# tooHotSpot/FGN

Hardware: AMD Instinct MI355X
Metric: query-imgs/sec (3-way 3-shot, 800x1333 FGN simple_test) (higher is better)
Workload: dtype f32; 1 GPU; cfg3: COCO2VOC 3-way 3-shot, query 3x800x1333, supports 9x3x256^2, ResNet-50-C4, R<=300 proposals, D<=100 detections, 1 episode(s) per GPU per step; h2d_in_step=True, gt_mask_rle_in_step=True, world_size_seen=1, phase_lock=rpn, caller_streams=2, support_cache=False, hip_graph=True, winograd_3x3=F(4x4,3x3)

## Files before the change

### fgn_amd/csrc/conv_igemm.hip

```cpp
#include "common.h"
#include <cstdlib>

struct ConvParams {
    const float* x = nullptr;
    const float* w = nullptr;
    float* y = nullptr;
    const float* scale = nullptr;
    const float* shift = nullptr;
    const float* residual = nullptr;
    const float* in_scale = nullptr;
    const int32_t* n_img_dev = nullptr;
    int n_img = 0, H = 1, W = 1, Cin = 0, Ho = 1, Wo = 1, Cout = 0, KH = 1, KW = 1, stride = 1, pad = 0;
    int a_img_div = 1;
    int relu = 0;
    int K = 0;
    int n_tiles_n = 0;
    int band_nt = 0, band_mt = 0;
    float* ws = nullptr;
    int splits = 1, kt_per_split = 0;
#ifdef FGN_EXPERIMENTS
    int32_t* tickets = nullptr;
    int32_t* sched = nullptr;
    int sk_U = 0, sk_dp = 0;
#endif
// ... 1152 lines not shown
    int tiles[2];
    const float* xs[2] = {x0, x1};
    float* ys[2] = {y0, y1};
    const int ns[2] = {n_img0, n_img1}, Hs[2] = {H0, H1}, Ws[2] = {W0, W1};
    for (int i = 0; i < 2; ++i) {
        const ConvPlan g = conv_geometry(ns[i], Hs[i], Ws[i], Cin, Cout, cout_pad, KH, KW, stride, pad, 1);
        if (g.rc != FGN_OK || g.x_bytes == 0) return FGN_ERR_SHAPE;
        ConvParams& p = ps[i];
        p.x = xs[i]; p.w = w_packed; p.y = ys[i]; p.scale = scale; p.shift = shift;
        p.n_img = ns[i]; p.H = Hs[i]; p.W = Ws[i]; p.Cin = Cin; p.Cout = Cout; p.KH = KH; p.KW = KW;
        p.stride = stride; p.pad = pad; p.relu = relu;
        p.Ho = g.Ho; p.Wo = g.Wo; p.K = g.K; p.x_bytes = g.x_bytes; p.w_bytes = g.w_bytes;
        p.kt_per_split = p.K / BK;
        p.n_tiles_n = cdiv(Cout, 64);
        const int m_tiles = cdiv((int)g.M, 64);
        set_band(p, 64, m_tiles, 64ll * p.K * 4);
        tiles[i] = (m_tiles * p.n_tiles_n + 7) / 8 * 8;
    }
    constexpr int NST = CONV_DMA_STAGES;
    const size_t dlds = std::max((size_t)NST * (64 + 64) * BK, (size_t)64 * (64 + 4)) * sizeof(float);
    const dim3 grid(tiles[0] + tiles[1]), wg(256);
    return Cin != 4 ? launch_kernel<conv_igemm_dma_pair_kernel<64, 64, 32, 32, NST, 4, 0>>(grid, wg, dlds, stream, ps[0], ps[1], tiles[0])
                    : launch_kernel<conv_igemm_dma_pair_kernel<64, 64, 32, 32, NST, 4, 2>>(grid, wg, dlds, stream, ps[0], ps[1], tiles[0]);
}

static int x3_pick_bm(long long M, int Cout, int K, int grp_rows, int grp_valid, int bm) {
    if (bm == 64 || bm == 128) return (grp_rows && grp_rows % bm) ? 0 : bm;
    if (grp_rows && grp_rows % 64) return 0;
    const int nt = cdiv(Cout, X3_BN);
    if (Cout * 10 < nt * X3_BN * 7) return 0;
    if (((M + 63) / 64) * nt < 192) return 0;
    const long long groups = grp_rows ? M / grp_rows : 1;
    const long long valid = grp_rows ? std::min<long long>(grp_valid > 0 ? grp_valid : grp_rows, grp_rows) : M;
    const long long rows64 = (valid + 63) / 64 * 64, rows128 = (valid + 127) / 128 * 128;
    if (K >= 256 && (!grp_rows || grp_rows % 128 == 0) && rows128 * 100 <= rows64 * 108 && groups * (rows128 / 128) * nt >= 400)
        return 128;
    return 64;
}

template <int WMW, int RB, int NT, int NST, bool SH16>
static int launch_x3_cfg(ConvParams& p, int M_max, hipStream_t stream) {
    constexpr int BM = 32 * RB * WMW;
    const int m_tiles = cdiv(M_max, BM);
    set_band(p, BM, m_tiles, (long long)X3_BN * p.K * 6);
    const int tiles = m_tiles * p.n_tiles_n;
    static unsigned long long ok = 0ull;
    hipError_t attr = fgn_allow_full_lds(reinterpret_cast<const void*>(conv_pw_x3_kernel<WMW, RB, NT, NST, SH16>), &ok);
    if (attr != hipSuccess) return (int)attr;
    const size_t lds = (size_t)NST * (BM * 128 + X3_B_STAGE);
    const int per_cu = (int)(160 * 1024 / lds);
    const int grid = std::min(256 * per_cu, (tiles + 7) / 8 * 8);
    p.stamp = fgn_next_stamp_record();
    FGN_LAUNCH_TIMED((conv_pw_x3_kernel<WMW, RB, NT, NST, SH16>), dim3(grid), dim3(128 * WMW), lds, stream, p, tiles);
    FGN_LAUNCH_CHECK();
    return FGN_OK;
}

static int launch_x3(const ConvParams& p0, int M_max, int bm, int nterms, hipStream_t stream) {
    ConvParams p = p0;
    if (!p.w3 || p.npad3 % X3_BN || p.npad3 < p.Cout || (p.Cout & 3) || p.K % BK || p.K < 2 * BK || p.splits != 1) return FGN_ERR_SHAPE;
    p.n_tiles_n = cdiv(p.Cout, X3_BN);
#ifdef FGN_EXPERIMENTS
    if (bm >= 2000) {
        const int b = bm - 2000;
        if (x3_pick_bm(M_max, p.Cout, p.K, p.grp_rows, p.grp_valid, b == 129 ? 128 : b) == 0) return FGN_ERR_SHAPE;
        if (b == 129) return nterms == 9 ? launch_x3_cfg<4, 1, 9, 3, false>(p, M_max, stream) : launch_x3_cfg<4, 1, 6, 3, false>(p, M_max, stream);
        if (b == 128) return launch_x3_cfg<2, 2, 6, 2, false>(p, M_max, stream);
        if (b == 64) return nterms == 9 ? launch_x3_cfg<2, 1, 9, 2, false>(p, M_max, stream) : launch_x3_cfg<2, 1, 6, 2, false>(p, M_max, stream);
        return FGN_ERR_SHAPE;
    }
#endif
    if (bm != 0 && bm != 64 && bm != 128) return FGN_ERR_SHAPE;
    const int BM = x3_pick_bm(M_max, p.Cout, p.K, p.grp_rows, p.grp_valid, bm);
    if (BM == 0) return FGN_ERR_SHAPE;
    if (nterms == 9) return BM == 64 ? launch_x3_cfg<2, 1, 9, 2, true>(p, M_max, stream) : FGN_ERR_SHAPE;
    return BM == 128 ? launch_x3_cfg<2, 2, 6, 2, true>(p, M_max, stream) : launch_x3_cfg<2, 1, 6, 2, true>(p, M_max, stream);
}

extern "C" size_t fgn_x3_image_bytes(int K, int npad, int n_groups) { return (size_t)n_groups * K * npad * 6; }
extern "C" int fgn_x3_row_tile(long long M, int Cout, int K, int grp_rows, int grp_valid) {
    return x3_pick_bm(M, Cout, K, grp_rows, grp_valid, 0);
}

#ifdef X3_PHASES
static unsigned long long* g_x3_ph = nullptr;
extern "C" int fgn_x3_phases(unsigned long long* host16) {
    if (!g_x3_ph) return FGN_ERR_ARG;
    if (hipDeviceSynchronize() != hipSuccess) return FGN_ERR_ARG;
    if (hipMemcpy(host16, g_x3_ph, 128, hipMemcpyDeviceToHost) != hipSuccess) return FGN_ERR_ARG;
    return hipMemset(g_x3_ph, 0, 128) == hipSuccess ? FGN_OK : FGN_ERR_ARG;
}
#endif

static int h2_pick(long long M, int Cout, int K, int grp_rows, int grp_valid, int bm) {
    if (bm == 264) return (grp_rows && grp_rows % 128) ? 0 : 264;
    if (bm != 0) return x3_pick_bm(M, Cout, K, grp_rows, grp_valid, bm);
    if (Cout <= 64) {
        if (grp_rows && grp_rows % 128) return 0;
        if (Cout < 48 || (M + 127) / 128 < 256) return 0;
        return 264;
    }
    const int bm_x3 = x3_pick_bm(M, Cout, K, grp_rows, grp_valid, 0);
    return (bm_x3 == 128 && !grp_rows) ? 64 : bm_x3;
}

template <int WMW, int WNW, int RB, int NST, bool IM2COL, int KG = 1>
static int launch_h2_cfg(ConvParams& p, const H2Im2col& q2, int M_max, hipStream_t stream) {
    constexpr int BM = 32 * RB * WMW, BN = 64 * WNW;
    const int m_tiles = cdiv(M_max, BM);
    p.n_tiles_n = cdiv(p.Cout, BN);
    set_band(p, BM, m_tiles, (long long)BN * p.K * 4);
    const int tiles = m_tiles * p.n_tiles_n;
    static unsigned long long ok = 0ull;
    hipError_t attr = fgn_allow_full_lds(reinterpret_cast<const void*>(conv_pw_h2_kernel<WMW, WNW, RB, NST, IM2COL, KG>), &ok);
    if (attr != hipSuccess) return (int)attr;
    const size_t lds = (size_t)KG * NST * (BM * 128 + 2 * BN * 64);
    const int per_cu = std::min(3, (int)(160 * 1024 / lds));
    const int grid = std::min(256 * per_cu, (tiles + 7) / 8 * 8);
    p.stamp = fgn_next_stamp_record();
    FGN_LAUNCH_TIMED((conv_pw_h2_kernel<WMW, WNW, RB, NST, IM2COL, KG>), dim3(grid), dim3(64 * WMW * WNW * KG), lds, stream, p, q2, tiles);
    FGN_LAUNCH_CHECK();
    return FGN_OK;
}

extern "C" size_t fgn_h2_image_bytes(int K, int npad, int n_groups) { return (size_t)n_groups * npad * ((size_t)K * 4 + 4); }
extern "C" int fgn_h2_row_tile(long long M, int Cout, int K, int grp_rows, int grp_valid) {
    return h2_pick(M, Cout, K, grp_rows, grp_valid, 0);
}

constexpr int H2_KG_MIN_KTILES = 8;
constexpr int H2_BM_KG2 = 1064;
extern "C" int fgn_h2_k_groups(long long M, int Cout, int K, int grp_rows, int grp_valid) {
    if (h2_pick(M, Cout, K, grp_rows, grp_valid, 0) != 64 || grp_rows != 0 || K % BK) return 1;
    const int kt = K / BK;
    if ((kt & 1) || kt < H2_KG_MIN_KTILES) return 1;
    return cdiv(M, 64) * (long long)cdiv(Cout, H2_BN) <= 256 ? 2 : 1;
}

static int launch_h2(const ConvParams& p0, int M_max, int n_groups, int bm, hipStream_t stream, const H2Im2col* im = nullptr) {
    ConvParams p = p0;
    if (!p.w3 || p.npad3 % H2_BN || p.npad3 < p.Cout || (p.Cout & 3) || p.K % BK || p.K < 2 * BK || p.splits != 1) return FGN_ERR_SHAPE;
    const size_t img = (size_t)n_groups * p.K * p.npad3 * 4;
    p.w3_bytes = (unsigned)img;
    p.w_inv = reinterpret_cast<const float*>(static_cast<const char*>(p.w3) + img);
    H2Im2col none;
    none.y1 = nullptr; none.x_off0 = none.x_off1 = 0u; none.M0 = none.M1 = 0; none.H1 = none.W1 = none.Ho1 = none.Wo1 = 1; none.cin_shift = 0;
    if (bm != 0 && bm != 64 && bm != 128 && bm != 264 && bm != H2_BM_KG2) return FGN_ERR_SHAPE;
    if (bm == H2_BM_KG2 && ((p.K / BK) % 2 || p.K / BK < 4)) return FGN_ERR_SHAPE;
    const int cfg = h2_pick(M_max, p.Cout, p.K, p.grp_rows, p.grp_valid, bm == H2_BM_KG2 ? 64 : bm);
    if (cfg == 0) return FGN_ERR_SHAPE;
    const int kgroups = bm == H2_BM_KG2 ? 2 : (bm == 0 ? fgn_h2_k_groups(M_max, p.Cout, p.K, p.grp_rows, p.grp_valid) : 1);
    if (kgroups == 2)
        return im ? launch_h2_cfg<2, 2, 1, 2, true, 2>(p, *im, M_max, stream) : launch_h2_cfg<2, 2, 1, 2, false, 2>(p, none, M_max, stream);
    if (im) {
        if (cfg == 264) return launch_h2_cfg<4, 1, 1, 2, true>(p, *im, M_max, stream);
        return cfg == 128 ? launch_h2_cfg<2, 2, 2, 2, true>(p, *im, M_max, stream) : launch_h2_cfg<2, 2, 1, 2, true>(p, *im, M_max, stream);
    }
    if (cfg == 264) return launch_h2_cfg<4, 1, 1, 2, false>(p, none, M_max, stream);
    return cfg == 128 ? launch_h2_cfg<2, 2, 2, 2, false>(p, none, M_max, stream) : launch_h2_cfg<2, 2, 1, 2, false>(p, none, M_max, stream);
}

extern "C" int fgn_conv2d_pair_h2_bm_nhwc_f32(const float* x0, int n_img0, int H0, int W0, const float* x1, int n_img1, int H1,
                                              int W1, const void* w_h2, float* y0, float* y1, const float* scale,
                                              const float* shift, int Cin, int Cout, int cout_pad, int KH, int KW, int stride,
                                              int pad, int relu, int bm, hipStream_t stream) {
    if (!x0 || !w_h2 || !y0 || (x1 && !y1)) return FGN_ERR_ARG;
    if (n_img0 <= 0 || (x1 && n_img1 <= 0)) return FGN_ERR_SHAPE;
// ... 90 lines not shown
                         int x2_total_rows, const void* w, float* y, const float* shift, int rows, int Cin1, int Cin2,
                         int Cout, int cout_pad, int relu) {
    if (!x || !x2 || !w || !y) return FGN_ERR_ARG;
    if (rows <= 0) return FGN_OK;
    if (Cin1 % BK || Cin2 % BK || Cin1 <= 0 || Cin2 <= 0 || (Cout & 3) || cout_pad % m.bn || cout_pad < Cout) return FGN_ERR_SHAPE;
    if ((!x2_rows && x2_total_rows != rows) || x2_total_rows < 1) return FGN_ERR_ARG;
    const long long K = (long long)Cin1 + Cin2;
    const long long xb = (long long)rows * Cin1 * 4, x2b = (long long)x2_total_rows * Cin2 * 4;
    const long long wb = gemm_weight_bytes(m, K, cout_pad, 1);
    if (xb >= 0x7fffff00ll || x2b >= 0x7fffff00ll || wb >= 0x7fffff00ll || (long long)rows * Cout >= (1ll << 31)) return FGN_ERR_SHAPE;
    p.x = x; p.y = y; p.shift = shift;
    p.x2 = x2; p.x2_bytes = (unsigned)x2b; p.kt1 = Cin1 / BK; p.cin2 = Cin2; p.x2_rows = x2_rows;
    p.n_img = rows; p.Cin = Cin1; p.Cout = Cout; p.relu = relu; p.K = (int)K;
    p.kt_per_split = (int)K / BK; p.x_bytes = (unsigned)xb;
    gemm_set_weights(p, m, w, wb, cout_pad);
    return FGN_DESCRIBED;
}

extern "C" int fgn_conv1x1_dual_nhwc_f32(const float* x, const float* x2, const int32_t* x2_rows, int x2_total_rows,
                                         const float* w_packed, float* y, const float* shift, int rows, int Cin1, int Cin2,
                                         int Cout, int cout_pad, int relu, hipStream_t stream) {
    ConvParams p;
    const int rc = describe_dual(p, MATH_F32, x, x2, x2_rows, x2_total_rows, w_packed, y, shift, rows, Cin1, Cin2, Cout, cout_pad, relu);
    if (rc != FGN_DESCRIBED) return rc;
    p.n_tiles_n = cdiv(Cout, 64);
    const int m_tiles = cdiv(rows, 64);
    set_band(p, 64, m_tiles, 64ll * p.K * 4);
    return launch_persist(p, m_tiles * p.n_tiles_n, stream);
}

extern "C" int fgn_conv1x1_dual_x3_nhwc_f32(const float* x, const float* x2, const int32_t* x2_rows, int x2_total_rows,
                                            const void* w_x3, float* y, const float* shift, int rows, int Cin1, int Cin2,
                                            int Cout, int cout_pad, int relu, hipStream_t stream) {
    ConvParams p;
    const int rc = describe_dual(p, MATH_X3, x, x2, x2_rows, x2_total_rows, w_x3, y, shift, rows, Cin1, Cin2, Cout, cout_pad, relu);
    if (rc != FGN_DESCRIBED) return rc;
    return launch_x3(p, rows, 0, 6, stream);
}

extern "C" int fgn_conv1x1_dual_h2_nhwc_f32(const float* x, const float* x2, const int32_t* x2_rows, int x2_total_rows,
                                            const void* w_h2, float* y, const float* shift, int rows, int Cin1, int Cin2,
                                            int Cout, int cout_pad, int relu, hipStream_t stream) {
    ConvParams p;
    const int rc = describe_dual(p, MATH_H2, x, x2, x2_rows, x2_total_rows, w_h2, y, shift, rows, Cin1, Cin2, Cout, cout_pad, relu);
    if (rc != FGN_DESCRIBED) return rc;
    return launch_h2(p, rows, 1, 0, stream);
}

static int describe_gemm(ConvParams& p, const GemmMath& m, const float* x, const void* w, float* y, const float* shift,
                         const float* residual, int rows, int K, int Cout, int npad, int relu, int grp_rows, int grp_valid,
                         int n_groups) {
    if (!x || !w || !y) return FGN_ERR_ARG;
    if (rows <= 0) return FGN_OK;
    if (K % BK || K <= 0 || (Cout & 3) || npad % m.bn || npad < Cout || n_groups < 1) return FGN_ERR_SHAPE;
    if (n_groups > 1 && (grp_rows <= 0 || (long long)n_groups * grp_rows != rows || grp_valid > grp_rows)) return FGN_ERR_SHAPE;
    const long long xb = (long long)rows * K * 4, wb = gemm_weight_bytes(m, K, npad, n_groups);
    if (xb >= 0x7fffff00ll || wb >= 0x7fffff00ll || (long long)rows * Cout >= (1ll << 31)) return FGN_ERR_SHAPE;
    p.x = x; p.y = y; p.shift = shift; p.residual = residual;
    p.n_img = rows; p.Cin = K; p.Cout = Cout; p.relu = relu; p.K = K; p.kt_per_split = K / BK; p.x_bytes = (unsigned)xb;
    p.grp_rows = n_groups > 1 ? grp_rows : 0; p.grp_valid = grp_valid;
    gemm_set_weights(p, m, w, wb, npad);
    return FGN_DESCRIBED;
}

extern "C" int fgn_gemm_x3_f32(const float* x, const void* w3, float* y, const float* shift, const float* residual,
                               int rows, int K, int Cout, int npad, int relu, int grp_rows, int grp_valid, int n_groups,
                               int bm, int nterms, hipStream_t stream) {
    ConvParams p;
    const int rc = describe_gemm(p, MATH_X3, x, w3, y, shift, residual, rows, K, Cout, npad, relu, grp_rows, grp_valid, n_groups);
    if (rc != FGN_DESCRIBED) return rc;
#ifdef X3_PHASES
    if (!g_x3_ph && (hipMalloc(&g_x3_ph, 128) != hipSuccess || hipMemset(g_x3_ph, 0, 128) != hipSuccess)) return FGN_ERR_ARG;
    p.ws = reinterpret_cast<float*>(g_x3_ph);
#endif
    return launch_x3(p, rows, bm, nterms, stream);
}

extern "C" int fgn_gemm_h2_f32(const float* x, const void* w_h2, float* y, const float* shift, const float* residual,
                               int rows, int K, int Cout, int npad, int relu, int grp_rows, int grp_valid, int n_groups,
                               int bm, hipStream_t stream) {
    ConvParams p;
    const int rc = describe_gemm(p, MATH_H2, x, w_h2, y, shift, residual, rows, K, Cout, npad, relu, grp_rows, grp_valid, n_groups);
    if (rc != FGN_DESCRIBED) return rc;
    return launch_h2(p, rows, n_groups, bm, stream);
}

extern "C" int fgn_winograd_t_pad(int tiles_total) { return (tiles_total + 127) / 128 * 128; }

static int describe_winograd_gemm(ConvParams& p, const GemmMath& m, const float* V, const void* U, float* Mo,
                                  const int32_t* n_img_dev, int n_img, int tiles_per_img, int t_pad, int Cin, int Cout,
                                  int cout_pad, int n_groups) {
    if (!V || !U || !Mo) return FGN_ERR_ARG;
    if (n_img <= 0) return FGN_OK;
    if (Cin % BK != 0 || (m.deep && Cin < 2 * BK) || Cout % 4 != 0 || cout_pad % m.bn != 0 || cout_pad < Cout || t_pad % 64 != 0 ||
        (n_groups != 16 && n_groups != 36) || (long long)n_img * tiles_per_img > t_pad)
        return FGN_ERR_SHAPE;
    const long long rows = (long long)n_groups * t_pad;
    const long long xb = rows * Cin * 4, wb = gemm_weight_bytes(m, Cin, cout_pad, n_groups);
    if (xb >= 0x7fffff00ll || wb >= 0x7fffff00ll || rows * Cout >= (1ll << 31)) return FGN_ERR_SHAPE;
    p.x = V; p.y = Mo;
    p.n_img = (int)rows; p.Cin = Cin; p.Cout = Cout; p.K = Cin; p.kt_per_split = Cin / BK; p.x_bytes = (unsigned)xb;
    p.grp_rows = t_pad; p.grp_valid = n_img * tiles_per_img; p.grp_items = n_img;
    p.grp_rows_per_item = tiles_per_img; p.grp_count_dev = n_img_dev;
    gemm_set_weights(p, m, U, wb, cout_pad);
    if (!m.image_bytes) p.grp_w_stride = cout_pad * Cin;
    return FGN_DESCRIBED;
}

extern "C" int fgn_winograd_gemm_f32(const float* V, const float* U, float* Mo, const int32_t* n_img_dev, int n_img,
                                     int tiles_per_img, int t_pad, int Cin, int Cout, int cout_pad, int n_groups,
                                     hipStream_t stream) {
    ConvParams p;
    const int rc = describe_winograd_gemm(p, MATH_F32, V, U, Mo, n_img_dev, n_img, tiles_per_img, t_pad, Cin, Cout, cout_pad, n_groups);
    if (rc != FGN_DESCRIBED) return rc;
#ifdef FGN_EXPERIMENTS
    {
        int rc2 = FGN_OK;
        if (fgn_exp_pointwise(p, p.n_img, 4, true, t_pad, stream, &rc2)) return rc2;
    }
#endif
    return launch_cfg<64, 64, 32, 32, 4>(p, p.n_img, pointwise_mode(4, p.n_img, Cout, 1), stream);
}

extern "C" int fgn_winograd_gemm_x3_f32(const float* V, const void* U_x3, float* Mo, const int32_t* n_img_dev, int n_img,
                                        int tiles_per_img, int t_pad, int Cin, int Cout, int cout_pad, int n_groups,
                                        hipStream_t stream) {
    ConvParams p;
    const int rc = describe_winograd_gemm(p, MATH_X3, V, U_x3, Mo, n_img_dev, n_img, tiles_per_img, t_pad, Cin, Cout, cout_pad, n_groups);
    if (rc != FGN_DESCRIBED) return rc;
    return launch_x3(p, p.n_img, 0, 6, stream);
}

extern "C" int fgn_winograd_gemm_h2_f32(const float* V, const void* U_h2, float* Mo, const int32_t* n_img_dev, int n_img,
                                        int tiles_per_img, int t_pad, int Cin, int Cout, int cout_pad, int n_groups,
                                        hipStream_t stream) {
    ConvParams p;
    const int rc = describe_winograd_gemm(p, MATH_H2, V, U_h2, Mo, n_img_dev, n_img, tiles_per_img, t_pad, Cin, Cout, cout_pad, n_groups);
    if (rc != FGN_DESCRIBED) return rc;
    return launch_h2(p, p.n_img, n_groups, 0, stream);
}
```

### fgn_amd/csrc/conv_pw_h2.h

```cpp
#pragma once

typedef _Float16 f16x8_t __attribute__((ext_vector_type(8)));

struct H2Frag { f16x8_t hi, lo; };

__device__ __forceinline__ void h2_split4(const float x0, const float x1, const float x2, const float x3, const float s,
                                          unsigned& h01, unsigned& h23, unsigned& l01, unsigned& l23) {
    asm("v_fma_mixlo_f16 %0, %4, %8, 0\n\t"
        "v_fma_mixlo_f16 %1, %6, %8, 0\n\t"
        "v_fma_mixhi_f16 %0, %5, %8, 0\n\t"
        "v_fma_mixhi_f16 %1, %7, %8, 0\n\t"
        "v_fma_mixlo_f16 %2, %4, %8, -%0 op_sel:[0,0,0] op_sel_hi:[0,0,1]\n\t"
        "v_fma_mixlo_f16 %3, %6, %8, -%1 op_sel:[0,0,0] op_sel_hi:[0,0,1]\n\t"
        "v_fma_mixhi_f16 %2, %5, %8, -%0 op_sel:[0,0,1] op_sel_hi:[0,0,1]\n\t"
        "v_fma_mixhi_f16 %3, %7, %8, -%1 op_sel:[0,0,1] op_sel_hi:[0,0,1]\n\t"
        "s_nop 1"
        : "=&v"(h01), "=&v"(h23), "=&v"(l01), "=&v"(l23)
        : "v"(x0), "v"(x1), "v"(x2), "v"(x3), "s"(s));
}

__device__ __forceinline__ H2Frag h2_split(const float4& a, const float4& b, const float s) {
    unsigned h[4], l[4];
    h2_split4(a.x, a.y, a.z, a.w, s, h[0], h[1], l[0], l[1]);
    h2_split4(b.x, b.y, b.z, b.w, s, h[2], h[3], l[2], l[3]);
    H2Frag f;
    f.hi = __builtin_bit_cast(f16x8_t, make_uint4(h[0], h[1], h[2], h[3]));
    f.lo = __builtin_bit_cast(f16x8_t, make_uint4(l[0], l[1], l[2], l[3]));
    return f;
}

__device__ __forceinline__ float h2_absmax16(const float4& a, const float4& b, const float4& c, const float4& d) {
    float m;
    asm("v_max3_f32 %0, |%1|, |%2|, 0\n\t"
        "v_max3_f32 %0, |%3|, |%4|, %0\n\t"
        "v_max3_f32 %0, |%5|, |%6|, %0\n\t"
        "v_max3_f32 %0, |%7|, |%8|, %0\n\t"
        "v_max3_f32 %0, |%9|, |%10|, %0\n\t"
        "v_max3_f32 %0, |%11|, |%12|, %0\n\t"
        "v_max3_f32 %0, |%13|, |%14|, %0\n\t"
        "v_max3_f32 %0, |%15|, |%16|, %0"
        : "=&v"(m)
        : "v"(a.x), "v"(a.y), "v"(a.z), "v"(a.w), "v"(b.x), "v"(b.y), "v"(b.z), "v"(b.w),
          "v"(c.x), "v"(c.y), "v"(c.z), "v"(c.w), "v"(d.x), "v"(d.y), "v"(d.z), "v"(d.w));
    return m;
}

constexpr int H2_BN = 128;

struct H2Im2col {
    float* y1;
    unsigned x_off0, x_off1;
    int M0, M1;
    int H1, W1, Ho1, Wo1;
    int cin_shift;
};

template <int WMW, int WNW, int RB, int NST, bool IM2COL, int KG = 1>
__global__ __launch_bounds__(64 * WMW * WNW * KG, KG == 1 ? 2 : 1) void conv_pw_h2_kernel(const ConvParams p, const H2Im2col q2, const int total_tiles) {
    constexpr int BM = 32 * RB * WMW, BN = 64 * WNW, NW = WMW * WNW, NTHR_G = 64 * NW, NTHR = NTHR_G * KG;
    static_assert(KG == 1 || KG == 2, "one or two K-groups");
    constexpr int A_LD = BM / 8 / NW;
    constexpr int A_STAGE = BM * 128;
    constexpr int B_STAGE = 2 * BN * 64;
    constexpr int STAGE = A_STAGE + B_STAGE;
    constexpr int BQ = BN / 16;
    constexpr int B_LD = 2 * BQ / NW;
    static_assert(A_LD * 8 * NW == BM && B_LD * NW == 2 * BQ, "tile / wave split");
    constexpr int PER = A_LD + B_LD;
    constexpr int D = NST - 1;
    constexpr int ROWS_PER_PASS = NTHR_G / 8;
    static_assert(NST == 2 || NST == 3, "ring of 2 or 3 stages");
    extern __shared__ __attribute__((aligned(16))) unsigned char smem_h2[];

    const int t = threadIdx.x, lane = t & 63;
    const int kg = KG == 1 ? 0 : __builtin_amdgcn_readfirstlane((t >> 6) / NW);
    const int wv = KG == 1 ? t >> 6 : (t >> 6) % NW;
    const int tg = KG == 1 ? t : t % NTHR_G;
    const int wm = wv / WNW, wn = wv % WNW;
    const int M = IM2COL ? q2.M0 + q2.M1 : (p.n_img_dev ? min(p.n_img, *p.n_img_dev) : p.n_img) * p.Ho * p.Wo;
    int grp_valid = p.grp_valid;
    if (p.grp_rows && p.grp_count_dev) grp_valid = min(grp_valid, min(p.grp_items, *p.grp_count_dev) * p.grp_rows_per_item);

    float a_s = 1.f, a_inv = 1.f;

    const int col4 = tg & 7, row0 = tg >> 3;
    const int src_c4 = col4 ^ ((row0 >> 1) & 7);
    const i32x4 x_rs = make_rsrc(p.x, p.x_bytes);
    const i32x4 w_rs = make_rsrc(p.w3, p.w3_bytes);
    const bool dual = !IM2COL && p.x2 != nullptr;
    const i32x4 x2_rs = make_rsrc(dual ? p.x2 : p.x, dual ? p.x2_bytes : p.x_bytes);
    const int KT = p.K / BK / KG;
    const unsigned kt_bytes = (unsigned)(2 * p.npad3 * 64);
    const unsigned lds_base = __builtin_amdgcn_readfirstlane((unsigned)reinterpret_cast<size_t>(smem_h2) + kg * (NST * STAGE));
    const unsigned wave_row_bytes = __builtin_amdgcn_readfirstlane(wv) * 8 * 128;
    constexpr unsigned OOB = 0x7ffffff0u;

    const int nq = total_tiles >> 3, nr = total_tiles & 7;
    auto coords = [&](int tile, int& m0, int& n0) -> bool {
        const int xcd = tile & 7, idx = tile >> 3;
        const int bid = (xcd < nr ? xcd * (nq + 1) : nr * (nq + 1) + (xcd - nr) * nq) + idx;
        int tile_m = bid / p.n_tiles_n;
        int tile_n = bid - tile_m * p.n_tiles_n;
        if (p.band_nt > 0) {
            const int per_grp = p.band_mt * p.n_tiles_n;
            const int grp = bid / per_grp;
            int r = bid - grp * per_grp;
            const int per_band = p.band_mt * p.band_nt;
            const int band = r / per_band;
            r -= band * per_band;
            const int mi = r / p.band_nt;
            tile_m = grp * p.band_mt + mi;
            tile_n = band * p.band_nt + (r - mi * p.band_nt);
        }
        m0 = tile_m * BM;
        n0 = tile_n * BN;
        if (m0 >= M) return false;
        if (p.grp_rows && m0 - (m0 / p.grp_rows) * p.grp_rows >= grp_valid) return false;
        return true;
    };
    auto next_active = [&](int tile, int& m0, int& n0) -> int {
        for (; tile < total_tiles; tile += gridDim.x)
            if (coords(tile, m0, n0)) return tile;
        return -1;
    };

    struct Offs { unsigned a[A_LD], a2[A_LD], b[B_LD]; };
    unsigned b_lds[B_LD];
#pragma unroll
    for (int i = 0; i < B_LD; ++i) {
        const int q = wv + NW * i;
        b_lds[i] = __builtin_amdgcn_readfirstlane((unsigned)(A_STAGE + (q / BQ) * (BN * 64) + (q % BQ) * 1024));
    }
    auto offsets = [&](int m0, int n0) -> Offs {
        Offs o;
        const int g_end = p.grp_rows ? (m0 / p.grp_rows) * p.grp_rows + grp_valid : M;
#pragma unroll
        for (int i = 0; i < A_LD; ++i) {
            const int m = m0 + row0 + ROWS_PER_PASS * i;
            if constexpr (IM2COL) {
                o.a[i] = 0u; o.a2[i] = 0u;
                if (m < M) {
                    const bool t1 = m >= q2.M0;
                    const int mm = t1 ? m - q2.M0 : m;
                    const int H = t1 ? q2.H1 : p.H, W = t1 ? q2.W1 : p.W, Wo = t1 ? q2.Wo1 : p.Wo;
                    const int HoWo = (t1 ? q2.Ho1 : p.Ho) * Wo;
                    const int img = mm / HoWo;
                    const int rem = mm - img * HoWo;
                    const int oy = rem / Wo;
                    const int ox = rem - oy * Wo;
                    const int iy0 = oy * p.stride - p.pad, ix0 = ox * p.stride - p.pad;
                    o.a[i] = (t1 ? q2.x_off1 : q2.x_off0) + (unsigned)((((img * H + iy0) * W + ix0) * p.Cin + src_c4 * 4) * 4);
                    unsigned tm = t1 ? 0x80000000u : 0u;
                    int tp = 0;
                    for (int ky = 0; ky < p.KH; ++ky) {
                        const bool y_ok = (unsigned)(iy0 + ky) < (unsigned)H;
                        for (int kx = 0; kx < p.KW; ++kx, ++tp)
                            if (y_ok && (unsigned)(ix0 + kx) < (unsigned)W) tm |= 1u << tp;
                    }
                    o.a2[i] = tm;
                }
                continue;
            }
            const bool in = m < M && m < g_end;
            o.a[i] = in ? (unsigned)((m * p.Cin + src_c4 * 4) * 4) : OOB;
            o.a2[i] = OOB;
            if (dual && in) o.a2[i] = (unsigned)(((p.x2_rows ? p.x2_rows[m] : m) * p.cin2 + src_c4 * 4) * 4);
        }
        unsigned g0 = 0;
        if (p.grp_rows) g0 = (unsigned)(m0 / p.grp_rows) * (unsigned)(KT * KG) * kt_bytes;
#pragma unroll
        for (int i = 0; i < B_LD; ++i) {
            const int q = wv + NW * i;
            const int plane = q / BQ, row = (q % BQ) * 16 + (lane >> 2);
            o.b[i] = g0 + (unsigned)(((plane * p.npad3 + n0 + row) * 4 + (lane & 3)) * 16);
        }
        return o;
    };
    auto issue = [&](const Offs& o, int step, int stage) {
        const int kt = step * KG + kg;
        const unsigned st = lds_base + stage * STAGE;
        const unsigned sa = st + wave_row_bytes;
        const unsigned ko = (unsigned)(kt * BK * 4);
        if constexpr (IM2COL) {
            const int tap = kt >> q2.cin_shift;
            const int c0 = (kt - (tap << q2.cin_shift)) * BK;
            const int ky = p.KW == 3 ? (tap * 43) >> 7 : tap;
            const int kx = tap - ky * p.KW;
            const unsigned off0 = (unsigned)(((ky * p.W + kx) * p.Cin + c0) * 4);
            const unsigned off1 = (unsigned)(((ky * q2.W1 + kx) * p.Cin + c0) * 4);
#pragma unroll
            for (int i = 0; i < A_LD; ++i) {
                const bool ok = (o.a2[i] >> tap) & 1u;
                const unsigned voff = ok ? o.a[i] + ((o.a2[i] >> 31) ? off1 : off0) : OOB;
                lds_dma16_s(x_rs, sa + i * ROWS_PER_PASS * 128, voff, 0u);
            }
        } else if (dual && kt >= p.kt1) {
            const unsigned ko2 = (unsigned)((kt - p.kt1) * BK * 4);
#pragma unroll
            for (int i = 0; i < A_LD; ++i) lds_dma16_s(x2_rs, sa + i * ROWS_PER_PASS * 128, o.a2[i], ko2);
        } else {
#pragma unroll
            for (int i = 0; i < A_LD; ++i) lds_dma16_s(x_rs, sa + i * ROWS_PER_PASS * 128, o.a[i], ko);
        }
        const unsigned kb = (unsigned)kt * kt_bytes;
#pragma unroll
        for (int i = 0; i < B_LD; ++i) lds_dma16_s(w_rs, st + b_lds[i], o.b[i], kb);
    };

    const int r16 = lane & 15, g4 = lane >> 4;
    const int a16_row = wm * 32 * RB + r16;
    const unsigned a16_sw = (unsigned)((a16_row >> 1) & 7);
    const unsigned a16_rd0 = (unsigned)(a16_row * 128) + ((((unsigned)g4) ^ a16_sw) << 4);
    const unsigned a16_rd1 = (unsigned)(a16_row * 128) + ((((unsigned)(g4 + 4)) ^ a16_sw) << 4);
    const int n16 = wn * 64 + r16;
    const unsigned tau16 = (0x1230u >> (4 * ((n16 >> 2) & 3))) & 3u;
    const unsigned b16_rd = (unsigned)(A_STAGE + n16 * 64) + ((((unsigned)g4) ^ tau16) << 4);

    if (p.stamp && t == 0 && blockIdx.x == 0) atomicExch(p.stamp, __builtin_amdgcn_s_memrealtime());
    auto leave = [&]() {
        if (!p.stamp || t != 0) return;
        const unsigned shard = blockIdx.x & 7u;
        const unsigned long long in_shard = (gridDim.x - shard + 7u) / 8u;
        unsigned long long* const sc = p.stamp + 8 * (1 + shard);
        if (atomicAdd(sc, 1ull) != in_shard - 1) return;
        atomicExch(sc, 0ull);
        const unsigned long long shards = gridDim.x < 8u ? gridDim.x : 8u;
        if (atomicAdd(p.stamp + 2, 1ull) != shards - 1) return;
        const unsigned long long d = __builtin_amdgcn_s_memrealtime() - atomicExch(p.stamp, 0ull);
        atomicExch(p.stamp + 2, 0ull);
        atomicAdd(p.stamp + 1, d);
        atomicAdd(p.stamp + 3, 1ull);
        atomicMin(p.stamp + 4, d);
        atomicMax(p.stamp + 5, d);
    };

    int m0, n0, nm0 = 0, nn0 = 0;
    int tile = next_active(blockIdx.x, m0, n0);
    if (tile < 0) { leave(); return; }
    Offs cur = offsets(m0, n0);
    int ntile = next_active(tile + gridDim.x, nm0, nn0);
    Offs nxt = cur;
    if (ntile >= 0) nxt = offsets(nm0, nn0);
    int ic_kt = 0, ic_stage = 0, ahead = 0;
    bool ic_next = false;
    auto issue_one = [&]() {
        if (!ic_next) {
            issue(cur, ic_kt, ic_stage);
            if (++ic_kt == KT) { ic_next = true; ic_kt = 0; }
        } else {
            if (ntile < 0 || ic_kt >= KT) return;
            issue(nxt, ic_kt, ic_stage);
            ++ic_kt;
        }
        ic_stage = ic_stage + 1 == NST ? 0 : ic_stage + 1;
        ++ahead;
    };
#pragma unroll
    for (int i = 0; i < D; ++i) issue_one();
    int stage = 0;

    while (true) {
        f32x4 acc[2 * RB][4];
#pragma unroll
        for (int i = 0; i < 2 * RB; ++i)
#pragma unroll
            for (int j = 0; j < 4; ++j) acc[i][j] = f32x4{0.f, 0.f, 0.f, 0.f};
        bool have_s = false;
        float a_lim = 0.f;
        a_s = 1.f; a_inv = 1.f;
        for (int kt = 0; kt < KT; ++kt) {
            if (D == 2 && kt > 0 && ahead == 2) x3_wait_vm<PER>(); else x3_wait_vm<0>();
            asm volatile("s_waitcnt lgkmcnt(0)" ::: "memory");
            __builtin_amdgcn_s_barrier();
            --ahead;
            issue_one();
            asm volatile("" ::: "memory");
            const unsigned char* const S = smem_h2 + (KG == 1 ? 0 : kg * (NST * STAGE)) + stage * STAGE;
            float4 alo[2 * RB], ahi[2 * RB];
            f16x8_t bq[4][2];
#pragma unroll
            for (int i = 0; i < 2 * RB; ++i) {
                alo[i] = *reinterpret_cast<const float4*>(S + a16_rd0 + i * (16 * 128));
                ahi[i] = *reinterpret_cast<const float4*>(S + a16_rd1 + i * (16 * 128));
            }
#pragma unroll
            for (int j = 0; j < 4; ++j)
#pragma unroll
                for (int q = 0; q < 2; ++q)
                    bq[j][q] = *reinterpret_cast<const f16x8_t*>(S + b16_rd + j * (16 * 64) + q * (BN * 64));
            __builtin_amdgcn_sched_barrier(0);
            auto adapt = [&]() {
                auto fin = [](const float v) { const float a = fabsf(v); return a < __builtin_inff() ? a : 0.f; };
                float m = 0.f;
#pragma unroll
                for (int i = 0; i < 2 * RB; ++i) {
                    m = fmaxf(m, fmaxf(fmaxf(fin(alo[i].x), fin(alo[i].y)), fmaxf(fin(alo[i].z), fin(alo[i].w))));
                    m = fmaxf(m, fmaxf(fmaxf(fin(ahi[i].x), fin(ahi[i].y)), fmaxf(fin(ahi[i].z), fin(ahi[i].w))));
                }
#pragma unroll
                for (int o = 32; o > 0; o >>= 1) m = fmaxf(m, __shfl_xor(m, o));
                const unsigned mb = __builtin_amdgcn_readfirstlane(__float_as_uint(m));
                const int e = (int)((mb >> 23) & 0xffu);
                if (e < 27) return;
                if (have_s && __uint_as_float(mb) <= a_lim) return;
                const float ns = __uint_as_float((unsigned)(267 - e) << 23);
                const float ratio = ns * a_inv;
                if (have_s) {
#pragma unroll
                    for (int i = 0; i < 2 * RB; ++i)
#pragma unroll
                        for (int j = 0; j < 4; ++j) acc[i][j] *= ratio;
                }
                a_s = ns;
                a_inv = __uint_as_float((unsigned)(e - 13) << 23);
                a_lim = 65504.f * a_inv;
                have_s = true;
            };
            {
                float big = h2_absmax16(alo[0], ahi[0], alo[1], ahi[1]);
                if constexpr (RB == 2) big = fmaxf(big, h2_absmax16(alo[2], ahi[2], alo[3], ahi[3]));
                if (__builtin_expect(__builtin_amdgcn_ballot_w64(!(big <= a_lim)) != 0ull, 0)) adapt();
            }
#pragma unroll
            for (int i = 0; i < 2 * RB; ++i) {
                const H2Frag a = h2_split(alo[i], ahi[i], a_s);
#pragma unroll
                for (int j = 0; j < 4; ++j) {
                    f32x4 c = acc[i][j];
                    c = __builtin_amdgcn_mfma_f32_16x16x32_f16(a.lo, bq[j][0], c, 0, 0, 0);
                    c = __builtin_amdgcn_mfma_f32_16x16x32_f16(a.hi, bq[j][1], c, 0, 0, 0);
                    c = __builtin_amdgcn_mfma_f32_16x16x32_f16(a.hi, bq[j][0], c, 0, 0, 0);
                    acc[i][j] = c;
                }
            }
            stage = stage + 1 == NST ? 0 : stage + 1;
        }
        float* const cbase = reinterpret_cast<float*>(smem_h2 + (stage == 0 ? NST - 1 : stage - 1) * STAGE);
        const int em0 = m0, en0 = n0;
        const float* const winv = p.w_inv + (p.grp_rows ? (size_t)(em0 / p.grp_rows) * p.npad3 : 0);
        constexpr int PR = 32 * RB;
#pragma unroll
        for (int pass = 0; pass < WMW; ++pass) {
            __syncthreads();
            if (wm == pass && kg == 0) {
#pragma unroll
                for (int i = 0; i < 2 * RB; ++i)
#pragma unroll
                    for (int j = 0; j < 4; ++j) {
                        float* cw = cbase + (16 * i + 4 * g4) * BN + wn * 64 + 16 * j + r16;
#pragma unroll
                        for (int r = 0; r < 4; ++r) cw[r * BN] = acc[i][j][r] * a_inv;
                    }
            }
            __syncthreads();
            if constexpr (KG == 2) {
                if (wm == pass && kg == 1) {
#pragma unroll
                    for (int i = 0; i < 2 * RB; ++i)
#pragma unroll
                        for (int j = 0; j < 4; ++j) {
                            float* cw = cbase + (16 * i + 4 * g4) * BN + wn * 64 + 16 * j + r16;
#pragma unroll
                            for (int r = 0; r < 4; ++r) cw[r * BN] += acc[i][j][r] * a_inv;
                        }
                }
                __syncthreads();
            }
            constexpr int C4 = BN / 4, RPP = NTHR / C4, NPASS = PR / RPP, SW = NPASS < 4 ? NPASS : 4;
            static_assert(NPASS % SW == 0, "row sweeps in groups of SW");
            const int c4 = t % C4, rr = t / C4;
            const int n = en0 + c4 * 4;
            if (n < p.Cout) {
                float4 sc = make_float4(1.f, 1.f, 1.f, 1.f), sh = make_float4(0.f, 0.f, 0.f, 0.f);
                if (p.scale) sc = *reinterpret_cast<const float4*>(p.scale + n);
                if (p.shift) sh = *reinterpret_cast<const float4*>(p.shift + n);
                const float4 iv = *reinterpret_cast<const float4*>(winv + n);
#pragma unroll
                for (int k0 = 0; k0 < NPASS; k0 += SW) {
                    float4 res[SW];
#pragma unroll
                    for (int k = 0; k < SW; ++k) {
                        const int m = em0 + PR * pass + rr + RPP * (k0 + k);
                        res[k] = make_float4(0.f, 0.f, 0.f, 0.f);
                        if (p.residual && m < M) res[k] = *reinterpret_cast<const float4*>(p.residual + (size_t)m * p.Cout + n);
                    }
#pragma unroll
                    for (int k = 0; k < SW; ++k) {
                        const int row = rr + RPP * (k0 + k);
                        const int m = em0 + PR * pass + row;
                        if (m >= M) continue;
                        float4 v = *reinterpret_cast<const float4*>(cbase + row * BN + c4 * 4);
                        v.x *= iv.x; v.y *= iv.y; v.z *= iv.z; v.w *= iv.w;
                        v.x = v.x * sc.x + sh.x; v.y = v.y * sc.y + sh.y; v.z = v.z * sc.z + sh.z; v.w = v.w * sc.w + sh.w;
                        v.x += res[k].x; v.y += res[k].y; v.z += res[k].z; v.w += res[k].w;
                        if (p.relu) {
                            v.x = fmaxf(v.x, 0.f); v.y = fmaxf(v.y, 0.f); v.z = fmaxf(v.z, 0.f); v.w = fmaxf(v.w, 0.f);
                        }
                        float* const yrow = (IM2COL && m >= q2.M0) ? q2.y1 + (size_t)(m - q2.M0) * p.Cout : p.y + (size_t)m * p.Cout;
                        *reinterpret_cast<float4*>(yrow + n) = v;
                    }
                }
            }
        }
        if (ntile < 0) break;
        tile = ntile; m0 = nm0; n0 = nn0;
        cur = nxt;
        ic_next = ic_kt >= KT;
        if (ic_next) ic_kt = 0;
        ntile = next_active(tile + gridDim.x, nm0, nn0);
        if (ntile >= 0) nxt = offsets(nm0, nn0);
    }
    asm volatile("s_waitcnt vmcnt(0)" ::: "memory");
    leave();
}
```

Baseline: 325.4 img/s.

## Restructure h2 pointwise GEMM K-loop with incremental cursor and interleaved fp16 split

After: 329.9 img/s, median of 6. 1.01x the previous value.

```diff
diff --git a/fgn_amd/csrc/conv_igemm.hip b/fgn_amd/csrc/conv_igemm.hip
--- a/fgn_amd/csrc/conv_igemm.hip
+++ b/fgn_amd/csrc/conv_igemm.hip
@@ -1258,7 +1258,7 @@
     return x3_pick_bm(M, Cout, K, grp_rows, grp_valid, 0);
 }
 
-#ifdef X3_PHASES
+#if defined(X3_PHASES) || defined(H2_PHASES)
 static unsigned long long* g_x3_ph = nullptr;
 extern "C" int fgn_x3_phases(unsigned long long* host16) {
     if (!g_x3_ph) return FGN_ERR_ARG;
@@ -1515,6 +1515,10 @@
     ConvParams p;
     const int rc = describe_gemm(p, MATH_H2, x, w_h2, y, shift, residual, rows, K, Cout, npad, relu, grp_rows, grp_valid, n_groups);
     if (rc != FGN_DESCRIBED) return rc;
+#ifdef H2_PHASES
+    if (!g_x3_ph && (hipMalloc(&g_x3_ph, 128) != hipSuccess || hipMemset(g_x3_ph, 0, 128) != hipSuccess)) return FGN_ERR_ARG;
+    p.ws = reinterpret_cast<float*>(g_x3_ph);
+#endif
     return launch_h2(p, rows, n_groups, bm, stream);
 }
 
diff --git a/fgn_amd/csrc/conv_pw_h2.h b/fgn_amd/csrc/conv_pw_h2.h
--- a/fgn_amd/csrc/conv_pw_h2.h
+++ b/fgn_amd/csrc/conv_pw_h2.h
@@ -17,6 +17,26 @@
         "s_nop 1"
         : "=&v"(h01), "=&v"(h23), "=&v"(l01), "=&v"(l23)
         : "v"(x0), "v"(x1), "v"(x2), "v"(x3), "s"(s));
+}
+
+__device__ __forceinline__ void h2_split4_step(const int step, const float x0, const float x1, const float x2, const float x3,
+                                               const float s, unsigned& h01, unsigned& h23, unsigned& l01, unsigned& l23) {
+    if (step == 0)
+        asm("v_fma_mixlo_f16 %0, %2, %4, 0\n\t"
+            "v_fma_mixlo_f16 %1, %3, %4, 0"
+            : "=&v"(h01), "=&v"(h23) : "v"(x0), "v"(x2), "s"(s));
+    else if (step == 1)
+        asm("v_fma_mixhi_f16 %0, %2, %4, 0\n\t"
+            "v_fma_mixhi_f16 %1, %3, %4, 0"
+            : "+v"(h01), "+v"(h23) : "v"(x1), "v"(x3), "s"(s));
+    else if (step == 2)
+        asm("v_fma_mixlo_f16 %0, %2, %4, -%5 op_sel:[0,0,0] op_sel_hi:[0,0,1]\n\t"
+            "v_fma_mixlo_f16 %1, %3, %4, -%6 op_sel:[0,0,0] op_sel_hi:[0,0,1]"
+            : "=&v"(l01), "=&v"(l23) : "v"(x0), "v"(x2), "s"(s), "v"(h01), "v"(h23));
+    else
+        asm("v_fma_mixhi_f16 %0, %2, %4, -%5 op_sel:[0,0,1] op_sel_hi:[0,0,1]\n\t"
+            "v_fma_mixhi_f16 %1, %3, %4, -%6 op_sel:[0,0,1] op_sel_hi:[0,0,1]"
+            : "+v"(l01), "+v"(l23) : "v"(x1), "v"(x3), "s"(s), "v"(h01), "v"(h23));
 }
 
 __device__ __forceinline__ H2Frag h2_split(const float4& a, const float4& b, const float s) {
@@ -55,6 +75,11 @@
     int cin_shift;
 };
 
+#ifdef H2_PHASES
+#define H2_T(i) do { const unsigned long long now_ = __builtin_amdgcn_s_memtime(); ph_[i] += now_ - last_; last_ = now_; } while (0)
+#else
+#define H2_T(i) do { } while (0)
+#endif
 template <int WMW, int WNW, int RB, int NST, bool IM2COL, int KG = 1>
 __global__ __launch_bounds__(64 * WMW * WNW * KG, KG == 1 ? 2 : 1) void conv_pw_h2_kernel(const ConvParams p, const H2Im2col q2, const int total_tiles) {
     constexpr int BM = 32 * RB * WMW, BN = 64 * WNW, NW = WMW * WNW, NTHR_G = 64 * NW, NTHR = NTHR_G * KG;
@@ -67,9 +92,9 @@
     constexpr int B_LD = 2 * BQ / NW;
     static_assert(A_LD * 8 * NW == BM && B_LD * NW == 2 * BQ, "tile / wave split");
     constexpr int PER = A_LD + B_LD;
-    constexpr int D = NST - 1;
     constexpr int ROWS_PER_PASS = NTHR_G / 8;
-    static_assert(NST == 2 || NST == 3, "ring of 2 or 3 stages");
+    constexpr bool OLD_CURSOR = KG == 2 && !IM2COL;
+    static_assert(NST == 2, "a ring of two stages: one K-tile in flight ahead of the one being multiplied");
     extern __shared__ __attribute__((aligned(16))) unsigned char smem_h2[];
 
     const int t = threadIdx.x, lane = t & 63;
@@ -176,25 +201,71 @@
         }
         return o;
     };
-    auto issue = [&](const Offs& o, int step, int stage) {
+    const unsigned ko_step = (unsigned)(KG * BK * 4), kb_step = (unsigned)KG * kt_bytes;
+    const unsigned ko1 = dual ? (unsigned)(p.kt1 * BK * 4) : 0xffffffffu;
+    unsigned c_ko = 0u, c_kb = 0u;
+    int c_tap = 0, c_cs = 0, c_kx = 0;
+    unsigned c_off0 = 0u, c_off1 = 0u;
+    const int im_ct = 1 << q2.cin_shift;
+    const unsigned im_skip0 = (unsigned)((p.W - p.KW) * p.Cin * 4), im_skip1 = (unsigned)((q2.W1 - p.KW) * p.Cin * 4);
+    auto seek = [&](int step) {
         const int kt = step * KG + kg;
-        const unsigned st = lds_base + stage * STAGE;
+        c_ko = (unsigned)(kt * BK * 4);
+        c_kb = (unsigned)kt * kt_bytes;
+        if constexpr (IM2COL) {
+            c_tap = kt >> q2.cin_shift;
+            c_cs = kt - (c_tap << q2.cin_shift);
+            const int ky = p.KW == 3 ? (c_tap * 43) >> 7 : c_tap;
+            c_kx = c_tap - ky * p.KW;
+            c_off0 = (unsigned)(((ky * p.W + c_kx) * p.Cin + c_cs * BK) * 4);
+            c_off1 = (unsigned)(((ky * q2.W1 + c_kx) * p.Cin + c_cs * BK) * 4);
+        }
+    };
+    auto advance = [&]() {
+        c_ko += ko_step;
+        c_kb += kb_step;
+        if constexpr (IM2COL) {
+#pragma unroll
+            for (int g = 0; g < KG; ++g) {
+                const bool tw = ++c_cs == im_ct;
+                c_cs = tw ? 0 : c_cs;
+                c_tap += tw;
+                c_kx += tw;
+                const bool rw = c_kx == p.KW;
+                c_kx = rw ? 0 : c_kx;
+                c_off0 += 128u + (rw ? im_skip0 : 0u);
+                c_off1 += 128u + (rw ? im_skip1 : 0u);
+            }
+        }
+    };
+    auto piece = [&](const Offs& o, const unsigned wr, const int idx) {
+        const unsigned st = lds_base + wr;
+        if (idx >= A_LD) {
+            const int i = idx - A_LD;
+            lds_dma16_s(w_rs, st + b_lds[i], o.b[i], c_kb);
+            return;
+        }
+        const int i = idx;
+        const unsigned dst = st + wave_row_bytes + i * ROWS_PER_PASS * 128;
+        if constexpr (IM2COL) {
+            const bool ok = (o.a2[i] >> c_tap) & 1u;
+            const unsigned voff = ok ? o.a[i] + ((o.a2[i] >> 31) ? c_off1 : c_off0) : OOB;
+            lds_dma16_s(x_rs, dst, voff, 0u);
+        } else {
+            const bool second = c_ko >= ko1;
+            i32x4 rs;
+            rs[0] = second ? x2_rs[0] : x_rs[0]; rs[1] = second ? x2_rs[1] : x_rs[1];
+            rs[2] = second ? x2_rs[2] : x_rs[2]; rs[3] = x_rs[3];
+            lds_dma16_s(rs, dst, second ? o.a2[i] : o.a[i], second ? c_ko - ko1 : c_ko);
+        }
+    };
+
+    auto issue_step = [&](const Offs& o, const int step, const unsigned wr) {
+        const int kt = step * KG + kg;
+        const unsigned st = lds_base + wr;
         const unsigned sa = st + wave_row_bytes;
         const unsigned ko = (unsigned)(kt * BK * 4);
-        if constexpr (IM2COL) {
-            const int tap = kt >> q2.cin_shift;
-            const int c0 = (kt - (tap << q2.cin_shift)) * BK;
-            const int ky = p.KW == 3 ? (tap * 43) >> 7 : tap;
-            const int kx = tap - ky * p.KW;
-            const unsigned off0 = (unsigned)(((ky * p.W + kx) * p.Cin + c0) * 4);
-            const unsigned off1 = (unsigned)(((ky * q2.W1 + kx) * p.Cin + c0) * 4);
-#pragma unroll
-            for (int i = 0; i < A_LD; ++i) {
-                const bool ok = (o.a2[i] >> tap) & 1u;
-                const unsigned voff = ok ? o.a[i] + ((o.a2[i] >> 31) ? off1 : off0) : OOB;
-                lds_dma16_s(x_rs, sa + i * ROWS_PER_PASS * 128, voff, 0u);
-            }
-        } else if (dual && kt >= p.kt1) {
+        if (dual && kt >= p.kt1) {
             const unsigned ko2 = (unsigned)((kt - p.kt1) * BK * 4);
 #pragma unroll
             for (int i = 0; i < A_LD; ++i) lds_dma16_s(x2_rs, sa + i * ROWS_PER_PASS * 128, o.a2[i], ko2);
@@ -239,25 +310,33 @@
     if (tile < 0) { leave(); return; }
     Offs cur = offsets(m0, n0);
     int ntile = next_active(tile + gridDim.x, nm0, nn0);
-    Offs nxt = cur;
-    if (ntile >= 0) nxt = offsets(nm0, nn0);
-    int ic_kt = 0, ic_stage = 0, ahead = 0;
+    auto following = [&]() -> Offs { return ntile >= 0 ? offsets(nm0, nn0) : cur; };
+    Offs nxt = following();
+    int ic_kt = 0;
     bool ic_next = false;
-    auto issue_one = [&]() {
+    auto issue_one = [&](const unsigned wr) {
         if (!ic_next) {
-            issue(cur, ic_kt, ic_stage);
+            issue_step(cur, ic_kt, wr);
             if (++ic_kt == KT) { ic_next = true; ic_kt = 0; }
         } else {
             if (ntile < 0 || ic_kt >= KT) return;
-            issue(nxt, ic_kt, ic_stage);
+            issue_step(nxt, ic_kt, wr);
             ++ic_kt;
         }
-        ic_stage = ic_stage + 1 == NST ? 0 : ic_stage + 1;
-        ++ahead;
-    };
-#pragma unroll
-    for (int i = 0; i < D; ++i) issue_one();
-    int stage = 0;
+    };
+    if constexpr (OLD_CURSOR) {
+        issue_one(0u);
+    } else {
+        seek(0);
+#pragma unroll
+        for (int i = 0; i < PER; ++i) piece(cur, 0u, i);
+        advance();
+    }
+    unsigned rd = 0u;
+#ifdef H2_PHASES
+    unsigned long long ph_[7] = {0, 0, 0, 0, 0, 0, 0}, last_ = __builtin_amdgcn_s_memtime();
+    const unsigned long long begin_ = last_;
+#endif
 
     while (true) {
         f32x4 acc[2 * RB][4];
@@ -268,14 +347,18 @@
         bool have_s = false;
         float a_lim = 0.f;
         a_s = 1.f; a_inv = 1.f;
-        for (int kt = 0; kt < KT; ++kt) {
-            if (D == 2 && kt > 0 && ahead == 2) x3_wait_vm<PER>(); else x3_wait_vm<0>();
+        auto k_tile = [&](auto&& requests) {
+            H2_T(5);
+            x3_wait_vm<0>();
             asm volatile("s_waitcnt lgkmcnt(0)" ::: "memory");
             __builtin_amdgcn_s_barrier();
-            --ahead;
-            issue_one();
             asm volatile("" ::: "memory");
-            const unsigned char* const S = smem_h2 + (KG == 1 ? 0 : kg * (NST * STAGE)) + stage * STAGE;
+            H2_T(0);
+            const unsigned wr = rd ^ (unsigned)STAGE;
+            requests(wr);
+            asm volatile("" ::: "memory");
+            H2_T(1);
+            const unsigned char* const S = smem_h2 + (KG == 1 ? 0 : kg * (NST * STAGE)) + rd;
             float4 alo[2 * RB], ahi[2 * RB];
             f16x8_t bq[4][2];
 #pragma unroll
@@ -289,6 +372,10 @@
                 for (int q = 0; q < 2; ++q)
                     bq[j][q] = *reinterpret_cast<const f16x8_t*>(S + b16_rd + j * (16 * 64) + q * (BN * 64));
             __builtin_amdgcn_sched_barrier(0);
+#ifdef H2_PHASES
+            asm volatile("s_waitcnt lgkmcnt(0)" ::: "memory");
+            H2_T(2);
+#endif
             auto adapt = [&]() {
                 auto fin = [](const float v) { const float a = fabsf(v); return a < __builtin_inff() ? a : 0.f; };
                 float m = 0.f;
@@ -321,21 +408,74 @@
                 if constexpr (RB == 2) big = fmaxf(big, h2_absmax16(alo[2], ahi[2], alo[3], ahi[3]));
                 if (__builtin_expect(__builtin_amdgcn_ballot_w64(!(big <= a_lim)) != 0ull, 0)) adapt();
             }
-#pragma unroll
-            for (int i = 0; i < 2 * RB; ++i) {
-                const H2Frag a = h2_split(alo[i], ahi[i], a_s);
-#pragma unroll
-                for (int j = 0; j < 4; ++j) {
-                    f32x4 c = acc[i][j];
-                    c = __builtin_amdgcn_mfma_f32_16x16x32_f16(a.lo, bq[j][0], c, 0, 0, 0);
-                    c = __builtin_amdgcn_mfma_f32_16x16x32_f16(a.hi, bq[j][1], c, 0, 0, 0);
-                    c = __builtin_amdgcn_mfma_f32_16x16x32_f16(a.hi, bq[j][0], c, 0, 0, 0);
-                    acc[i][j] = c;
-                }
-            }
-            stage = stage + 1 == NST ? 0 : stage + 1;
-        }
-        float* const cbase = reinterpret_cast<float*>(smem_h2 + (stage == 0 ? NST - 1 : stage - 1) * STAGE);
+            if constexpr (RB == 2 || OLD_CURSOR) {
+#pragma unroll
+                for (int i = 0; i < 2 * RB; ++i) {
+                    const H2Frag a = h2_split(alo[i], ahi[i], a_s);
+#ifdef H2_PHASES
+                    if (i == 0) { asm volatile("s_nop 0" ::"v"(a.hi), "v"(a.lo)); H2_T(3); }
+#endif
+#pragma unroll
+                    for (int j = 0; j < 4; ++j) {
+                        f32x4 c = acc[i][j];
+                        c = __builtin_amdgcn_mfma_f32_16x16x32_f16(a.lo, bq[j][0], c, 0, 0, 0);
+                        c = __builtin_amdgcn_mfma_f32_16x16x32_f16(a.hi, bq[j][1], c, 0, 0, 0);
+                        c = __builtin_amdgcn_mfma_f32_16x16x32_f16(a.hi, bq[j][0], c, 0, 0, 0);
+                        acc[i][j] = c;
+                    }
+                }
+            } else {
+                unsigned fh[2][4], fl[2][4];
+                h2_split4(alo[0].x, alo[0].y, alo[0].z, alo[0].w, a_s, fh[0][0], fh[0][1], fl[0][0], fl[0][1]);
+                h2_split4(ahi[0].x, ahi[0].y, ahi[0].z, ahi[0].w, a_s, fh[0][2], fh[0][3], fl[0][2], fl[0][3]);
+#ifdef H2_PHASES
+                asm volatile("s_nop 0" ::"v"(fh[0][0]), "v"(fl[0][3]));
+                H2_T(3);
+#endif
+#pragma unroll
+                for (int i = 0; i < 2 * RB; ++i) {
+                    const int u = i & 1, v = u ^ 1;
+                    const f16x8_t a_hi = __builtin_bit_cast(f16x8_t, make_uint4(fh[u][0], fh[u][1], fh[u][2], fh[u][3]));
+                    const f16x8_t a_lo = __builtin_bit_cast(f16x8_t, make_uint4(fl[u][0], fl[u][1], fl[u][2], fl[u][3]));
+                    const int n = i + 1 < 2 * RB ? i + 1 : i;
+#pragma unroll
+                    for (int j = 0; j < 4; ++j) {
+                        f32x4 c = acc[i][j];
+#pragma unroll
+                        for (int m = 0; m < 3; ++m) {
+                            c = __builtin_amdgcn_mfma_f32_16x16x32_f16(m == 0 ? a_lo : a_hi, bq[j][m == 1 ? 1 : 0], c, 0, 0, 0);
+                            if (m < 2 && i + 1 < 2 * RB) {
+                                const int sn = 2 * j + m, half = sn >> 2;
+                                const float4& x = half == 0 ? alo[n] : ahi[n];
+                                h2_split4_step(sn & 3, x.x, x.y, x.z, x.w, a_s, fh[v][2 * half], fh[v][2 * half + 1],
+                                               fl[v][2 * half], fl[v][2 * half + 1]);
+                            }
+                            __builtin_amdgcn_sched_barrier(0);
+                        }
+                        acc[i][j] = c;
+                    }
+                }
+            }
+#ifdef H2_PHASES
+            asm volatile("s_nop 0" ::"v"(acc[0][0][0]), "v"(acc[2 * RB - 1][3][3]));
+            H2_T(4);
+            ++ph_[6];
+#endif
+            if constexpr (!OLD_CURSOR) advance();
+            rd = wr;
+        };
+        auto request = [&](const Offs& o, const unsigned wr) {
+#pragma unroll
+            for (int k = 0; k < PER; ++k) piece(o, wr, k);
+        };
+        if constexpr (OLD_CURSOR) {
+            for (int kt = 0; kt < KT; ++kt) k_tile([&](const unsigned wr) { issue_one(wr); });
+        } else {
+            for (int kt = 0; kt < KT - 1; ++kt) k_tile([&](const unsigned wr) { request(cur, wr); });
+            seek(0);
+            k_tile([&](const unsigned wr) { if (ntile >= 0) request(nxt, wr); });
+        }
+        float* const cbase = reinterpret_cast<float*>(smem_h2 + (rd ^ (unsigned)STAGE));
         const int em0 = m0, en0 = n0;
         const float* const winv = p.w_inv + (p.grp_rows ? (size_t)(em0 / p.grp_rows) * p.npad3 : 0);
         constexpr int PR = 32 * RB;
@@ -405,11 +545,20 @@
         if (ntile < 0) break;
         tile = ntile; m0 = nm0; n0 = nn0;
         cur = nxt;
-        ic_next = ic_kt >= KT;
-        if (ic_next) ic_kt = 0;
+        if constexpr (OLD_CURSOR) {
+            ic_next = ic_kt >= KT;
+            if (ic_next) ic_kt = 0;
+        }
         ntile = next_active(tile + gridDim.x, nm0, nn0);
-        if (ntile >= 0) nxt = offsets(nm0, nn0);
+        nxt = following();
     }
     asm volatile("s_waitcnt vmcnt(0)" ::: "memory");
+#ifdef H2_PHASES
+    if (p.ws && lane == 0 && wv == 0 && kg == 0 && blockIdx.x < 2) {
+        unsigned long long* o = reinterpret_cast<unsigned long long*>(p.ws) + 8 * blockIdx.x;
+        for (int i = 0; i < 7; ++i) o[i] = ph_[i];
+        o[7] = __builtin_amdgcn_s_memtime() - begin_;
+    }
+#endif
     leave();
 }
```
